# rakhimovv/lvt

Hardware: AMD Instinct MI355X
Metric: video-clips/sec/node (VQVAE+DSFVT train step, BAIR 64x64x16) (higher is better)
Workload: dtype f32

## Files before the change

lvt_amd/csrc/epilogue_fast.h:

```cpp
#pragma once
#include "lvt_common.h"

typedef float lvt_f32x16 __attribute__((ext_vector_type(16)));

template <int TM, int TN>
__device__ __forceinline__ void lvt_f16x2_finish(lvt_f32x16 (&acc)[TM][TN], lvt_f32x16 (&acx)[TM][TN], int unscale) {
    if (unscale >= -100 && unscale <= 120) {
        const float s = __uint_as_float((unsigned)(unscale + 127) << 23), sx = __uint_as_float((unsigned)(unscale + 116) << 23);
#pragma unroll
        for (int i = 0; i < TM; ++i)
#pragma unroll
            for (int j = 0; j < TN; ++j) acc[i][j] = acx[i][j] * sx + acc[i][j] * s;
    } else {
#pragma unroll
        for (int i = 0; i < TM; ++i)
#pragma unroll
            for (int j = 0; j < TN; ++j)
#pragma unroll
                for (int r = 0; r < 16; ++r) acc[i][j][r] = ldexpf(fmaf(acx[i][j][r], 1.f / 2048.f, acc[i][j][r]), unscale);
    }
}

struct LvtEpi {
    int M, N;
    float *C; long long ldc;
    long long coff;
    float alpha; int flags;
    const float *bias; const float *res; long long ldr; const float *mask; long long ldm;
};

struct LvtRowIdentity {
    static constexpr int LANE_STEP = 1;
    __device__ __forceinline__ long long operator()(int row) const { return row; }
};

template <int F, int TM, int TN, class RM = LvtRowIdentity>
__device__ __forceinline__ float lvt_epi_fast_wave(const LvtEpi &e, lvt_f32x16 (&acc)[TM][TN], float *wave_tile, int m_w, int n_w,
                                                   int lane, const RM rm = RM()) {
#pragma clang fp contract(off)
    static_assert(TM == 2 && TN == 2, "64 x 64 sub-tiles");
    constexpr int SW = TN * 32;
    const int flags = F >= 0 ? F : e.flags;
    const bool f_bias = flags & LVT_EPI_BIAS, f_res = flags & LVT_EPI_RESIDUAL, f_relu = flags & LVT_EPI_RELU, f_mask = flags & LVT_EPI_MASK;
    const bool f_leaky = flags & LVT_EPI_LEAKY, f_lkm = flags & LVT_EPI_LEAKY_MASK;
    const int l31 = lane & 31, half = lane >> 5;
    const int c4 = lane & 15, r0 = lane >> 4;
    const int col = n_w + 4 * c4;
    const bool colok = col < e.N;
    float4 bias4 = make_float4(0.f, 0.f, 0.f, 0.f);
    if (f_bias && colok) bias4 = *reinterpret_cast<const float4 *>(e.bias + col);
    float am = 0.f;
    long long orow_all[TM][8];
    float4 rv_all[TM][8], mv_all[TM][8];
#pragma unroll
    for (int i = 0; i < TM; ++i) {
        const int row0 = m_w + i * 32 + r0;
#pragma unroll
        for (int u = 0; u < 8; ++u) orow_all[i][u] = rm(row0 + 4 * u);
    }
    auto request = [&](int i) {
        const int row0 = m_w + i * 32 + r0;
        if (f_res) {
            const float *rp = e.res + e.coff + col;
#pragma unroll
            for (int u = 0; u < 8; ++u)
                rv_all[i][u] = (colok && row0 + 4 * u < e.M) ? *reinterpret_cast<const float4 *>(rp + orow_all[i][u] * e.ldr) : make_float4(0.f, 0.f, 0.f, 0.f);
        }
        if (f_mask) {
            const float *mp = e.mask + e.coff + col;
#pragma unroll
            for (int u = 0; u < 8; ++u)
                mv_all[i][u] = (colok && row0 + 4 * u < e.M) ? *reinterpret_cast<const float4 *>(mp + orow_all[i][u] * e.ldm) : make_float4(0.f, 0.f, 0.f, 0.f);
        }
    };
#pragma unroll
    for (int i = 0; i < TM; ++i) request(i);
#pragma unroll
    for (int i = 0; i < TM; ++i) {
#pragma unroll
        for (int j = 0; j < TN; ++j)
#pragma unroll
            for (int r = 0; r < 16; ++r) wave_tile[((r & 3) + 8 * (r >> 2) + 4 * half) * SW + 32 * j + l31] = acc[i][j][r];
        const int row0 = m_w + i * 32 + r0;
        const long long (&orow)[8] = orow_all[i];
        const float4 (&rv)[8] = rv_all[i];
        const float4 (&mv)[8] = mv_all[i];
        float *cp = e.C + e.coff + col;
#pragma unroll
        for (int u = 0; u < 8; ++u) {
            float4 v = *reinterpret_cast<const float4 *>(&wave_tile[(r0 + 4 * u) * SW + 4 * c4]);
            v.x *= e.alpha; v.y *= e.alpha; v.z *= e.alpha; v.w *= e.alpha;
            if (f_bias) { v.x += bias4.x; v.y += bias4.y; v.z += bias4.z; v.w += bias4.w; }
            if (f_res) { v.x += rv[u].x; v.y += rv[u].y; v.z += rv[u].z; v.w += rv[u].w; }
            if (f_relu) { v.x = fmaxf(v.x, 0.f); v.y = fmaxf(v.y, 0.f); v.z = fmaxf(v.z, 0.f); v.w = fmaxf(v.w, 0.f); }
            if (f_leaky) { v.x = lvt_leakyf(v.x); v.y = lvt_leakyf(v.y); v.z = lvt_leakyf(v.z); v.w = lvt_leakyf(v.w); }
            if (f_mask) { v.x = lvt_maskf(v.x, mv[u].x, f_lkm); v.y = lvt_maskf(v.y, mv[u].y, f_lkm); v.z = lvt_maskf(v.z, mv[u].z, f_lkm); v.w = lvt_maskf(v.w, mv[u].w, f_lkm); }
            if (colok && row0 + 4 * u < e.M) {
                am = fmaxf(am, fmaxf(fmaxf(lvt_absf(v.x), lvt_absf(v.y)), fmaxf(lvt_absf(v.z), lvt_absf(v.w))));
                *reinterpret_cast<float4 *>(cp + orow[u] * e.ldc) = v;
            }
        }
    }
    return am;
}

typedef __attribute__((address_space(1))) char lvt_gchar;
typedef float lvt_f32x4 __attribute__((ext_vector_type(4)));
typedef __attribute__((address_space(1))) lvt_f32x4 lvt_gf32x4;
__device__ __forceinline__ lvt_gchar *lvt_sgpr_ptr(lvt_gchar *p) { asm("" : "+s"(p)); return p; }
template <int F, int TM, int TN, class RM>
__device__ __forceinline__ float lvt_epi_lean_wave(const LvtEpi &e, lvt_f32x16 (&acc)[TM][TN], float *wave_tile, int m_w, int n_w, int lane,
                                                   const RM rm) {
#pragma clang fp contract(off)
    static_assert(F >= 0 && TM == 2 && TN == 2, "compile-time flags, 64 x 64 sub-tiles");
    constexpr int SW = TN * 32;
    constexpr bool f_bias = F & LVT_EPI_BIAS, f_res = F & LVT_EPI_RESIDUAL, f_relu = F & LVT_EPI_RELU, f_mask = F & LVT_EPI_MASK;
    constexpr bool f_leaky = F & LVT_EPI_LEAKY, f_lkm = F & LVT_EPI_LEAKY_MASK;
    const int l31 = lane & 31, half = lane >> 5;
    const int c4 = lane & 15, r0 = lane >> 4;
    const unsigned loff = (unsigned)(RM::LANE_STEP * r0) * (unsigned)e.ldc * 4u + 16u * c4;
    const unsigned ld4 = (unsigned)e.ldc * 4u;
    const long long first = (e.coff + n_w + rm(m_w) * e.ldc) * 4;
    lvt_f32x4 bias4 = {0.f, 0.f, 0.f, 0.f};
    if (f_bias) bias4 = *(const lvt_gf32x4 *)((lvt_gchar *)(e.bias + n_w) + 16u * c4);
    unsigned rowb[TM][8];
#pragma unroll
    for (int i = 0; i < TM; ++i)
#pragma unroll
        for (int u = 0; u < 8; ++u) rowb[i][u] = (unsigned)(rm(m_w + 32 * i + 4 * u) - rm(m_w)) * ld4;
    lvt_gchar *Cb = (lvt_gchar *)e.C + first;
    lvt_gchar *Rb = f_res ? (lvt_gchar *)e.res + first : nullptr;
    lvt_gchar *Mb = f_mask ? (lvt_gchar *)e.mask + first : nullptr;
    lvt_f32x4 rv[TM][8], mv[TM][8];
#pragma unroll
    for (int i = 0; i < TM; ++i) {
        if (f_res) {
#pragma unroll
            for (int u = 0; u < 8; ++u) rv[i][u] = *(const lvt_gf32x4 *)(lvt_sgpr_ptr(Rb + rowb[i][u]) + loff);
        }
        if (f_mask) {
#pragma unroll
            for (int u = 0; u < 8; ++u) mv[i][u] = *(const lvt_gf32x4 *)(lvt_sgpr_ptr(Mb + rowb[i][u]) + loff);
        }
    }
    auto key = [](float x) { return (__float_as_uint(x) << 1) + (1u << 24); };
    unsigned am = 1u << 24;
#pragma unroll
    for (int i = 0; i < TM; ++i) {
#pragma unroll
        for (int j = 0; j < TN; ++j)
#pragma unroll
            for (int r = 0; r < 16; ++r) wave_tile[((r & 3) + 8 * (r >> 2) + 4 * half) * SW + 32 * j + l31] = acc[i][j][r];
#pragma unroll
        for (int u = 0; u < 8; ++u) {
            lvt_f32x4 v = *reinterpret_cast<const lvt_f32x4 *>(&wave_tile[(r0 + 4 * u) * SW + 4 * c4]);
            if (f_bias) v += bias4;
            if (f_res) v += rv[i][u];
            if (f_relu) { v.x = fmaxf(v.x, 0.f); v.y = fmaxf(v.y, 0.f); v.z = fmaxf(v.z, 0.f); v.w = fmaxf(v.w, 0.f); }
            if (f_leaky) { v.x = lvt_leakyf(v.x); v.y = lvt_leakyf(v.y); v.z = lvt_leakyf(v.z); v.w = lvt_leakyf(v.w); }
            if (f_mask) { v.x = lvt_maskf(v.x, mv[i][u].x, f_lkm); v.y = lvt_maskf(v.y, mv[i][u].y, f_lkm); v.z = lvt_maskf(v.z, mv[i][u].z, f_lkm); v.w = lvt_maskf(v.w, mv[i][u].w, f_lkm); }
            am = max(max(am, key(v.x)), key(v.y));
            am = max(max(am, key(v.z)), key(v.w));
            *(lvt_gf32x4 *)(lvt_sgpr_ptr(Cb + rowb[i][u]) + loff) = v;
        }
    }
    return __uint_as_float((am - (1u << 24)) >> 1);
}

__device__ __forceinline__ bool lvt_epi_lean_ok(const LvtEpi &e) {
    return e.alpha == 1.f && (unsigned long long)e.ldc < (1ull << 20) && (!(e.flags & LVT_EPI_RESIDUAL) || e.ldr == e.ldc) &&
           (!(e.flags & LVT_EPI_MASK) || e.ldm == e.ldc);
}
template <int F, int TM, int TN, class RM = LvtRowIdentity>
__device__ __forceinline__ float lvt_epi_fast_pick(const LvtEpi &e, lvt_f32x16 (&acc)[TM][TN], float *wave_tile, int m_w, int n_w, int lane,
                                                   const RM rm = RM()) {
    if constexpr (F >= 0) {
        const int m_u = __builtin_amdgcn_readfirstlane(m_w), n_u = __builtin_amdgcn_readfirstlane(n_w);
        if (lvt_epi_lean_ok(e) && m_u + TM * 32 <= e.M && n_u + TN * 32 <= e.N)
            return lvt_epi_lean_wave<F, TM, TN, RM>(e, acc, wave_tile, m_u, n_u, lane, rm);
    }
    return lvt_epi_fast_wave<F, TM, TN, RM>(e, acc, wave_tile, m_w, n_w, lane, rm);
}

template <int TM, int TN, class RM = LvtRowIdentity>
__device__ __forceinline__ float lvt_epi_fast_dispatch(const LvtEpi &e, lvt_f32x16 (&acc)[TM][TN], float *wave_tile, int m_w, int n_w, int lane,
                                                       const RM rm = RM()) {
#define LVT_EPI_CASE(F) case (F): return lvt_epi_fast_pick<(F), TM, TN, RM>(e, acc, wave_tile, m_w, n_w, lane, rm)
    switch (e.flags & (LVT_EPI_BIAS | LVT_EPI_RESIDUAL | LVT_EPI_RELU | LVT_EPI_MASK | LVT_EPI_LEAKY | LVT_EPI_LEAKY_MASK)) {
    LVT_EPI_CASE(0);
    LVT_EPI_CASE(LVT_EPI_BIAS);
    LVT_EPI_CASE(LVT_EPI_BIAS | LVT_EPI_RELU);
    LVT_EPI_CASE(LVT_EPI_BIAS | LVT_EPI_RESIDUAL);
    LVT_EPI_CASE(LVT_EPI_BIAS | LVT_EPI_RESIDUAL | LVT_EPI_RELU);
    LVT_EPI_CASE(LVT_EPI_RESIDUAL);
    LVT_EPI_CASE(LVT_EPI_MASK);
    LVT_EPI_CASE(LVT_EPI_RESIDUAL | LVT_EPI_MASK);
    LVT_EPI_CASE(LVT_EPI_BIAS | LVT_EPI_LEAKY);
    LVT_EPI_CASE(LVT_EPI_MASK | LVT_EPI_LEAKY_MASK);
    default: return lvt_epi_fast_wave<-1, TM, TN, RM>(e, acc, wave_tile, m_w, n_w, lane, rm);
    }
#undef LVT_EPI_CASE
}

__device__ __forceinline__ unsigned lvt_amax_peek(const float *dst) {
    return (dst && threadIdx.x == 0) ? __hip_atomic_load(reinterpret_cast<const unsigned *>(dst), __ATOMIC_RELAXED, __HIP_MEMORY_SCOPE_AGENT) : 0u;
}
__device__ __forceinline__ void lvt_block_amax_commit_seen(float m, float *dst, float *scratch, unsigned seen) {
#pragma unroll
    for (int d = 32; d > 0; d >>= 1) m = fmaxf(m, __shfl_xor(m, d, 64));
    const int nw = (blockDim.x + 63) >> 6;
    if ((threadIdx.x & 63) == 0) scratch[threadIdx.x >> 6] = m;
    __syncthreads();
    if (threadIdx.x == 0) {
        for (int w = 1; w < nw; ++w) m = fmaxf(m, scratch[w]);
        const unsigned bits = __float_as_uint(m);
        if (bits > seen) atomicMax(reinterpret_cast<unsigned *>(dst), bits);
    }
}
```

lvt_amd/csrc/gemm_engine.hip:

```cpp
#include "lvt_common.h"
#include "epilogue_fast.h"
#include <string.h>
#include <stdlib.h>
#include <stdint.h>
#include <type_traits>

typedef float f32x16 __attribute__((ext_vector_type(16)));

#define BK 32
#define NTHREADS 256

enum { A_KPLAIN = 0, A_MPLAIN = 1, A_CONV_K = 2, A_CONVT_K = 3, A_CONV_M = 4, A_ONEHOT_M = 5, A_PATCH = 6, A_PATCHT = 7 };
enum { B_KPLAIN = 0, B_NPLAIN = 1, B_CONVT_W = 2 };

struct KParams {
    int M, N, K;
    const float *A; long long lda; int a_kb; long long a_skb;
    const float *B; long long ldb; int b_kb; long long b_skb;
    float *C; long long ldc; long long c_plane;
    int batch_inner;
    long long sA_o, sA_i, sB_o, sB_i, sC_o, sC_i;
    float alpha; int flags;
    const float *bias; const float *res; long long ldr; const float *mask; long long ldm;
    int splits; int k_per_split; float *partial; long long partial_stride;
// ... 630 lines not shown
            long long orow = row;
            if (AMODE == A_PATCH) orow = patch_orow(row);
            if (AMODE == A_PATCHT) orow = patcht_orow(row, cls);
            if (AMODE == A_CONVT_K) {
                const lvt_conv_geom &g = p.g;
                int m = row;
                const int qw = m % p.Wq; m /= p.Wq;
                const int qh = m % p.Hq; m /= p.Hq;
                const int qt = m % p.Tq; const int n = m / p.Tq;
                orow = (((long long)n * g.Ti + (g.st * qt + rt)) * g.Hi + (g.sh * qh + rh)) * g.Wi +
                       (g.sw * qw + rw);
            }
#pragma unroll
            for (int j = 0; j < TN; ++j) {
                const int col = n0 + wn * (TN * 32) + j * 32 + l31;
                if (col >= p.N) continue;
                float v = acc[i][j][r];
                if (p.splits > 1) {
                    p.partial[split * p.partial_stride + (long long)z * p.M * p.N + orow * p.N + col] = v;
                    continue;
                }
                v *= p.alpha;
                if (flags & LVT_EPI_BIAS) v += p.bias[col];
                if (flags & LVT_EPI_RESIDUAL) v += p.res[coff + orow * p.ldr + col];
                if (flags & LVT_EPI_RELU) v = fmaxf(v, 0.f);
                if (flags & LVT_EPI_LEAKY) v = lvt_leakyf(v);
                if (flags & LVT_EPI_TANH) v = tanhf(v);
                if (flags & LVT_EPI_SIGMOID) v = lvt_sigmoid_col(v, col < p.N - LVT_EPI_PAD_OF(flags));
                if (flags & LVT_EPI_MASK) v = lvt_maskf(v, p.mask[coff + orow * p.ldm + col], flags & LVT_EPI_LEAKY_MASK);
                float *cp = p.C + coff + orow * p.ldc + col;
                if (flags & LVT_EPI_ACCUM) v += *cp;
                *cp = v;
                am = fmaxf(am, lvt_absf(v));
            }
        }
    }
    if (p.c_amax && p.splits <= 1) {
        __shared__ float amax_scratch[8];
        lvt_block_amax_commit(am, p.c_amax, amax_scratch);
    }
}

struct TileCtx { int m0, n0, z, split, cls, kbeg, kend; const float *A, *B; long long coff; };
template <int AMODE, int BM, int BN>
__device__ __forceinline__ TileCtx lvt_tile_ctx(const KParams &p) {
    TileCtx t;
    const int ntn = (p.N + BN - 1) / BN;
    int wg = blockIdx.x;
    t.split = blockIdx.z;
    t.z = blockIdx.y;
    if (p.splits > 1 && ((gridDim.y * gridDim.z) & 7) == 0) {
        const unsigned lin = blockIdx.x + gridDim.x * (blockIdx.y + gridDim.y * blockIdx.z);
        const unsigned xcd = lin & 7, slot = lin >> 3;
        const unsigned grp = xcd + 8 * (slot / gridDim.x);
        t.z = (int)(grp % gridDim.y);
        t.split = (int)(grp / gridDim.y);
        wg = (int)(slot % gridDim.x);
    } else {
        const int nwg = gridDim.x, q = nwg >> 3, r = nwg & 7;
        const int xcd = wg & 7, slot = wg >> 3;
        wg = (xcd < r ? xcd * (q + 1) : r * (q + 1) + (xcd - r) * q) + slot;
    }
    t.n0 = (wg % ntn) * BN; t.m0 = (wg / ntn) * BM;
    t.A = p.A; t.B = p.B; t.coff = 0; t.cls = 0;
    if (AMODE == A_CONVT_K) {
        t.cls = t.z;
    } else {
        const int zo = t.z / p.batch_inner, zi = t.z % p.batch_inner;
        t.A += zo * p.sA_o + zi * p.sA_i;
        t.B += zo * p.sB_o + zi * p.sB_i;
        t.coff = zo * p.sC_o + zi * p.sC_i;
    }
    t.kbeg = 0; t.kend = p.K;
    if (p.splits > 1) {
        t.kbeg = t.split * p.k_per_split;
        t.kend = min(p.K, t.kbeg + p.k_per_split);
    }
    if (p.flags & LVT_CAUSAL_KMAX) t.kend = min(t.kend, t.m0 + BM);
    if (p.flags & LVT_CAUSAL_KMIN) t.kbeg = max(t.kbeg, (t.m0 / BK) * BK);
    if ((p.flags & LVT_CAUSAL_TILE) && t.n0 > t.m0 + BM - 1) t.kend = t.kbeg;
    return t;
}

template <int AMODE, int BM, int BN, int WM, int WN>
__device__ __forceinline__ void lvt_epilogue_vec(const KParams &p, f32x16 (&acc)[BM / WM / 32][BN / WN / 32], float *lds,
                                                 int m0, int n0, int wm, int wn, int lane, int cls, long long coff, int z,
                                                 int split) {
#pragma clang fp contract(off)
    constexpr int TM = BM / WM / 32, TN = BN / WN / 32;
    constexpr int SW = TN * 32;
    constexpr int C4 = SW / 4;
    const int l31 = lane & 31, half = lane >> 5;
    float *tile = lds + (wm * WN + wn) * (32 * SW);
    int rt = 0, rh = 0, rw = 0;
    if (AMODE == A_CONVT_K) {
        const lvt_conv_geom &g = p.g;
        const int fw = cls % g.sw, fh = (cls / g.sw) % g.sh, ft = cls / (g.sw * g.sh);
        rt = ((ft - g.pt) % g.st + g.st) % g.st;
        rh = ((fh - g.ph) % g.sh + g.sh) % g.sh;
        rw = ((fw - g.pw) % g.sw + g.sw) % g.sw;
    }
    const int flags = p.flags;
    const bool lkm = flags & LVT_EPI_LEAKY_MASK;
    float am = 0.f;
#pragma unroll
    for (int i = 0; i < TM; ++i) {
#pragma unroll
        for (int j = 0; j < TN; ++j)
#pragma unroll
            for (int r = 0; r < 16; ++r) tile[((r & 3) + 8 * (r >> 2) + 4 * half) * SW + 32 * j + l31] = acc[i][j][r];
        __syncthreads();
        if (AMODE != A_KPLAIN && AMODE != A_MPLAIN && p.splits <= 1 && (flags & LVT_EPI_MASK) &&
            !(flags & (LVT_EPI_PLANES | LVT_EPI_ACCUM | LVT_EPI_LEAKY | LVT_EPI_LEAKY_MASK))) {
            constexpr int NU = 32 * C4 / 64;
            long long oaddr[NU];
            int ocol[NU];
#pragma unroll
            for (int u = 0; u < NU; ++u) {
                const int idx = lane + 64 * u;
                const int rowl = idx / C4, c4 = idx % C4;
                const int row = m0 + wm * (TM * 32) + i * 32 + rowl;
                const int col = n0 + wn * SW + 4 * c4;
                ocol[u] = col;
                long long orow = -1;
                if (row < p.M && col < p.N) {
                    orow = row;
                    if (AMODE == A_PATCH) orow = patch_orow(row);
                    if (AMODE == A_PATCHT) orow = patcht_orow(row, cls);
                    if (AMODE == A_CONVT_K) {
                        const lvt_conv_geom &g = p.g;
                        int m = row;
                        const int qw = m % p.Wq; m /= p.Wq;
                        const int qh = m % p.Hq; m /= p.Hq;
                        const int qt = m % p.Tq; const int n = m / p.Tq;
                        orow = (((long long)n * g.Ti + (g.st * qt + rt)) * g.Hi + (g.sh * qh + rh)) * g.Wi + (g.sw * qw + rw);
                    }
                }
                oaddr[u] = orow;
            }
            float4 rv[NU], mv[NU];
            if (flags & LVT_EPI_RESIDUAL) {
#pragma unroll
                for (int u = 0; u < NU; ++u) rv[u] = oaddr[u] >= 0 ? ldg4(p.res + coff + oaddr[u] * p.ldr + ocol[u]) : zero4();
            } else {
#pragma unroll
                for (int u = 0; u < NU; ++u) rv[u] = zero4();
            }
#pragma unroll
            for (int u = 0; u < NU; ++u) mv[u] = oaddr[u] >= 0 ? ldg4(p.mask + coff + oaddr[u] * p.ldm + ocol[u]) : zero4();
#pragma unroll
            for (int u = 0; u < NU; ++u) {
                const int idx = lane + 64 * u;
                const int rowl = idx / C4, c4 = idx % C4;
                const int col = ocol[u];
                const long long orow = oaddr[u];
                if (orow >= 0) {
                    float4 v = *reinterpret_cast<const float4 *>(&tile[rowl * SW + 4 * c4]);
                    v.x *= p.alpha; v.y *= p.alpha; v.z *= p.alpha; v.w *= p.alpha;
                    if (flags & LVT_EPI_BIAS) { const float4 b = ldg4(p.bias + col); v.x += b.x; v.y += b.y; v.z += b.z; v.w += b.w; }
                    v.x += rv[u].x; v.y += rv[u].y; v.z += rv[u].z; v.w += rv[u].w;
                    if (flags & LVT_EPI_RELU) { v.x = fmaxf(v.x, 0.f); v.y = fmaxf(v.y, 0.f); v.z = fmaxf(v.z, 0.f); v.w = fmaxf(v.w, 0.f); }
                    if (flags & LVT_EPI_TANH) { v.x = tanhf(v.x); v.y = tanhf(v.y); v.z = tanhf(v.z); v.w = tanhf(v.w); }
                    if (flags & LVT_EPI_SIGMOID) {
                        const int nr = p.N - LVT_EPI_PAD_OF(flags) - col;
                        v.x = lvt_sigmoid_col(v.x, nr > 0); v.y = lvt_sigmoid_col(v.y, nr > 1); v.z = lvt_sigmoid_col(v.z, nr > 2); v.w = lvt_sigmoid_col(v.w, nr > 3);
                    }
                    v.x = mv[u].x > 0.f ? v.x : 0.f; v.y = mv[u].y > 0.f ? v.y : 0.f; v.z = mv[u].z > 0.f ? v.z : 0.f; v.w = mv[u].w > 0.f ? v.w : 0.f;
                    am = fmaxf(am, fmaxf(fmaxf(lvt_absf(v.x), lvt_absf(v.y)), fmaxf(lvt_absf(v.z), lvt_absf(v.w))));
                    *reinterpret_cast<float4 *>(p.C + coff + orow * p.ldc + col) = v;
                }
            }
        } else {
#pragma unroll
            for (int u = 0; u < 32 * C4 / 64; ++u) {
                const int idx = lane + 64 * u;
                const int rowl = idx / C4, c4 = idx % C4;
                const int row = m0 + wm * (TM * 32) + i * 32 + rowl;
                const int col = n0 + wn * SW + 4 * c4;
                if (row < p.M && col < p.N) {
                    float4 v = *reinterpret_cast<const float4 *>(&tile[rowl * SW + 4 * c4]);
                    long long orow = row;
                    if (AMODE == A_PATCH) orow = patch_orow(row);
                    if (AMODE == A_PATCHT) orow = patcht_orow(row, cls);
                    if (AMODE == A_CONVT_K) {
                        const lvt_conv_geom &g = p.g;
                        int m = row;
                        const int qw = m % p.Wq; m /= p.Wq;
                        const int qh = m % p.Hq; m /= p.Hq;
                        const int qt = m % p.Tq; const int n = m / p.Tq;
                        orow = (((long long)n * g.Ti + (g.st * qt + rt)) * g.Hi + (g.sh * qh + rh)) * g.Wi + (g.sw * qw + rw);
                    }
                    if (p.splits > 1) {
                        *reinterpret_cast<float4 *>(p.partial + split * p.partial_stride + (long long)z * p.M * p.N + orow * p.N + col) = v;
// ... 159 lines not shown
                        acx[i][j] = __builtin_amdgcn_mfma_f32_32x32x16_f16(a[1][i], b[0][j], acx[i][j], 0, 0, 0);
            }
        } else {
            const unsigned short *Arh[TM], *Brh[TN];
#pragma unroll
            for (int i = 0; i < TM; ++i) Arh[i] = Ah + hrow<BM>(wm * (TM * 32) + i * 32 + l31) + 8 * half;
#pragma unroll
            for (int j = 0; j < TN; ++j) Brh[j] = Bh + hrow<BN>(wn * (TN * 32) + j * 32 + l31) + 8 * half;
#pragma unroll
            for (int ks = 0; ks < BK; ks += 16) {
                bf16x8 a[3][TM], b[3][TN];
#pragma unroll
                for (int q = 0; q < 3; ++q) {
#pragma unroll
                    for (int i = 0; i < TM; ++i)
                        a[q][i] = *reinterpret_cast<const bf16x8 *>(Arh[i] + q * PSA + ks);
#pragma unroll
                    for (int j = 0; j < TN; ++j)
                        b[q][j] = *reinterpret_cast<const bf16x8 *>(Brh[j] + q * PSB + ks);
                }
                constexpr int TA[6] = {1, 0, 2, 0, 1, 0}, TB[6] = {1, 2, 0, 1, 0, 0};
#pragma unroll
                for (int t = 0; t < 6; ++t)
#pragma unroll
                    for (int i = 0; i < TM; ++i)
#pragma unroll
                        for (int j = 0; j < TN; ++j)
                            acc[i][j] = __builtin_amdgcn_mfma_f32_32x32x16_bf16(a[TA[t]][i], b[TB[t]][j], acc[i][j], 0, 0, 0);
            }
        }
        __syncthreads();
        if (has_next) {
            if (MATH == 0) { al.store(As); bl.store(Bs); }
            else if (MATH == 1) { al.store_split(Ah); bl.store_split(Bh); }
            else { al.store_split2(Ah, sa); bl.store_split2(Bh, sb); }
        }
        __syncthreads();
    }
    if constexpr (MATH == 2) lvt_f16x2_finish<TM, TN>(acc, acx, unscale);

    if constexpr (COLSUM) {
        if (bl.sum_on) bl.write_colsum(lds, p.colsum_partial + (long long)split * p.N, n0, p.N, tid);
    }
    if constexpr (COLSUM_A) {
        if (al.sum_on) al.write_colsum(lds, p.colsum_partial + ((long long)split * gridDim.y + z) * p.M, m0, p.M, tid);
    }
    if constexpr (AMODE != A_CONVT_K && TM == 2 && TN == 2 && LDS_FLOATS >= TURN_FLOATS + 16) {
        if (p.vec_epi && !(p.flags & (LVT_EPI_PLANES | LVT_EPI_ACCUM | LVT_EPI_TANH | LVT_EPI_SIGMOID))) {
            LvtEpi e;
            e.M = p.M; e.N = p.N;
            float *wave_tile = lds + wave * (32 * TN * 32);
            if (COLSUM || COLSUM_A) __syncthreads();
            if (p.splits > 1) {
                e.C = p.partial; e.ldc = p.N; e.coff = split * p.partial_stride + (long long)z * p.M * p.N; e.alpha = 1.f; e.flags = 0;
                e.bias = nullptr; e.res = nullptr; e.ldr = 0; e.mask = nullptr; e.ldm = 0;
                (void)lvt_epi_fast_pick<0, TM, TN>(e, acc, wave_tile, m0 + wm * (TM * 32), n0 + wn * (TN * 32), lane);
                return;
            }
            const unsigned seen = lvt_amax_peek(p.c_amax);
            e.C = p.C; e.ldc = p.ldc; e.coff = coff; e.alpha = p.alpha; e.flags = p.flags;
            e.bias = p.bias; e.res = p.res; e.ldr = p.ldr; e.mask = p.mask; e.ldm = p.ldm;
            const float am_w = lvt_epi_fast_dispatch<TM, TN>(e, acc, wave_tile, m0 + wm * (TM * 32), n0 + wn * (TN * 32), lane);
            if (p.c_amax) lvt_block_amax_commit_seen(am_w, p.c_amax, lds + TURN_FLOATS, seen);
            return;
        }
    }
    if (p.vec_epi) lvt_epilogue_vec<AMODE, BM, BN, WM, WN>(p, acc, lds, m0, n0, wm, wn, lane, cls, coff, z, split);
    else lvt_epilogue<AMODE, BM, BN, WM, WN>(p, acc, m0, n0, wm, wn, l31, half, cls, coff, z, split);
}

#define PT_PW 18
#define PT_PIX (PT_PW * PT_PW)
#define PT_PLANE (PT_PIX * HLD)
#define PT_THREADS 512
typedef __attribute__((address_space(3))) void pt_lds_void;
typedef __attribute__((address_space(1))) const void pt_gl_void;
#define PT_BIMG_BYTES (2 * HPlane<128>::SIZE * 2)
template <int MODE, int MATH, int BIMG = 0>
__global__ __launch_bounds__(PT_THREADS) void lvt_conv_patch_kernel(const KParams p) {
    static_assert(!BIMG || MATH == 2, "weight images are f16x2 planes");
    constexpr int BM = 256, BN = 128, WM = 4, WN = 2, TM = 2, TN = 2;
    constexpr int NTAPS = MODE == 0 ? 9 : 4;
    constexpr int NP = MATH == 2 ? 2 : 3;
    constexpr int PSB = HPlane<BN>::SIZE;
    constexpr bool DBLA = MATH == 2;
    constexpr int A_IMG = NP * PT_PLANE;
    constexpr int A_BYTES = A_IMG * 2 * (DBLA ? 2 : 1), B_BYTES = NP * PSB * 2;
    constexpr int STAGE_FLOATS = (A_BYTES + 2 * B_BYTES) / 4 + 8;
    constexpr int TURN_FLOATS = WM * WN * 32 * (TN * 32);
    constexpr int LDS_FLOATS = STAGE_FLOATS > TURN_FLOATS ? STAGE_FLOATS : TURN_FLOATS;
    __shared__ __attribute__((aligned(16))) float lds[LDS_FLOATS];
    unsigned short *Ah = reinterpret_cast<unsigned short *>(lds);
    unsigned short *Bh0 = Ah + A_IMG * (DBLA ? 2 : 1);
    int unscale = 0;
    float sa = 1.f, sb = 1.f;
    if (MATH == 2) { sa = lvt_f16_scale(p.a_amax, unscale); sb = lvt_f16_scale(p.b_amax, unscale); }

    const int tid = threadIdx.x, lane = tid & 63, wave = tid >> 6;
    const int wm = wave / WN, wn = wave % WN;
    const int l31 = lane & 31, half = lane >> 5;
    const int Ci = p.g.Ci;
    const int ntn = p.N / BN;
    int wg = blockIdx.x;
    {
        const int nwg = gridDim.x, q = nwg >> 3, r = nwg & 7;
        const int xcd = wg & 7, slot = wg >> 3;
        wg = (xcd < r ? xcd * (q + 1) : r * (q + 1) + (xcd - r) * q) + slot;
    }
    const int n0 = (wg % ntn) * BN;
    const int frame = MODE == 1 ? (wg / ntn) >> 2 : wg / ntn, phase = MODE == 1 ? (wg / ntn) & 3 : 0, m0 = frame * BM;
    const float *xf = p.A + (long long)frame * (MODE == 2 ? 1024 : 256) * Ci;

    constexpr int PWALK = MODE == 2 ? 17 : PT_PW;
    constexpr int PUNITS = PWALK * PWALK * 8, PPASS = (PUNITS + PT_THREADS - 1) / PT_THREADS;
    float4 pv[PPASS];
    auto patch_fetch = [&](int chunk) {
#pragma unroll
        for (int j = 0; j < PPASS; ++j) {
            const int u = tid + PT_THREADS * j;
            const int pp = u >> 3, q = u & 7;
            const int py = pp / PWALK, px = pp - py * PWALK;
            if (MODE == 2) {
                const int iy = 2 * py + ((chunk >> 1) & 1) - 1, ix = 2 * px + (chunk & 1) - 1;
                const bool ok = u < PUNITS && (unsigned)iy < 32u && (unsigned)ix < 32u;
                pv[j] = ok ? ldg4(xf + (iy * 32 + ix) * Ci + (chunk >> 2) * 32 + q * 4) : zero4();
            } else {
                const bool ok = u < PUNITS && (unsigned)(py - 1) < 16u && (unsigned)(px - 1) < 16u;
                const float *src = xf + ((py - 1) * 16 + (px - 1)) * Ci + chunk * 32 + q * 4;
                pv[j] = ok ? ldg4(src) : zero4();
            }
        }
    };
    auto patch_store = [&](unsigned short *img) {
#pragma unroll
        for (int j = 0; j < PPASS; ++j) {
            const int u = tid + PT_THREADS * j;
            if (u < PUNITS) {
                const int pp = u >> 3;
                unsigned short *d = img + (MODE == 2 ? pp + pp / PWALK : pp) * HLD + (u & 7) * 4;
                if (MATH == 2) {
                    uint2 ph, pl;
                    split2(pv[j], sa, ph, pl);
                    *reinterpret_cast<uint2 *>(d) = ph;
                    *reinterpret_cast<uint2 *>(d + PT_PLANE) = pl;
                } else {
                    uint2 p1, p2, p3;
                    split3(pv[j], p1, p2, p3);
                    *reinterpret_cast<uint2 *>(d) = p1;
                    *reinterpret_cast<uint2 *>(d + PT_PLANE) = p2;
                    *reinterpret_cast<uint2 *>(d + 2 * PT_PLANE) = p3;
                }
            }
        }
    };
    const bool bact = tid < 256;
    const int bkk0 = (tid >> 5) & 7, bnq = tid & 31;
    const float *bcol = p.B + n0 + bnq * 4;
    float4 bv[4];
    auto b_fetch = [&](int step) {
        const int cc = step / NTAPS, tap = step - cc * NTAPS;
        const int wrow = MODE == 2 ? ((cc & 3) * NTAPS + tap) * Ci + (cc >> 2) * 32 : (phase * NTAPS + tap) * Ci + cc * 32;
        const float *src = bcol + (long long)(wrow + bkk0 * 4) * p.ldb;
#pragma unroll
        for (int i = 0; i < 4; ++i) bv[i] = ldg4(src + (long long)i * p.ldb);
    };

    f32x16 acc[TM][TN];
    f32x16 acx[MATH == 2 ? TM : 1][MATH == 2 ? TN : 1];
#pragma unroll
    for (int i = 0; i < TM; ++i)
#pragma unroll
        for (int j = 0; j < TN; ++j)
#pragma unroll
            for (int r = 0; r < 16; ++r) {
                acc[i][j][r] = 0.f;
                if (MATH == 2) acx[i][j][r] = 0.f;
            }
    auto b_store = [&](unsigned short *dst) {
        if (MATH == 2) store_split2_block<BN>(dst, bnq * 4, bkk0 * 4, bv, sb);
        else store_split_block<BN>(dst, bnq * 4, bkk0 * 4, bv);
    };
    const int wave_s = __builtin_amdgcn_readfirstlane(wave);
    constexpr int B_UNITS = PT_BIMG_BYTES / 16;
    static_assert(PT_BIMG_BYTES == NP * PSB * 2 || !BIMG, "image = the LDS buffer");
    const char *bimg0 = BIMG ? p.b_img + (long long)(n0 / BN) * PT_BIMG_BYTES + tid * 16 : nullptr;
    auto b_dma = [&](int step, unsigned short *dst) {
        const int cc = step / NTAPS, tap = step - cc * NTAPS;
        const int wrow = MODE == 2 ? ((cc & 3) * NTAPS + tap) * Ci + (cc >> 2) * 32 : (phase * NTAPS + tap) * Ci + cc * 32;
        const char *src = bimg0 + (long long)(wrow >> 5) * ntn * PT_BIMG_BYTES;
        char *d = reinterpret_cast<char *>(dst) + wave_s * 1024;
        __builtin_amdgcn_global_load_lds((pt_gl_void *)src, (pt_lds_void *)d, 16, 0, 0);
        __builtin_amdgcn_global_load_lds((pt_gl_void *)(src + 8192), (pt_lds_void *)(d + 8192), 16, 0, 0);
        if (tid + 1024 < B_UNITS) __builtin_amdgcn_global_load_lds((pt_gl_void *)(src + 16384), (pt_lds_void *)(d + 16384), 16, 0, 0);
    };
    const int b_nprobe = wave_s * 64 + 1024 < B_UNITS ? 3 : 2;
    const unsigned b_probe = (unsigned)((lane % b_nprobe) * 8192 + wave_s * 1024 + (lane & 31) * 16);
    auto b_landed = [&](const unsigned short *dst) {
        asm volatile("s_waitcnt vmcnt(0)" ::: "memory");
        const int v = *reinterpret_cast<const volatile int *>(reinterpret_cast<const char *>(dst) + b_probe);
        (void)v;
        asm volatile("s_waitcnt lgkmcnt(0)" ::: "memory");
    };

    int arow[TM];
    {
        const int q = l31 >> 2, e = l31 & 3;
        const int yy = __popc(q) & 1, x = 4 * (q >> 1) + e;
#pragma unroll
        for (int i = 0; i < TM; ++i) arow[i] = ((2 * (2 * wm + i) + yy) * PT_PW + x) * HLD + 8 * half;
    }
    int brow[TN];
#pragma unroll
    for (int j = 0; j < TN; ++j) brow[j] = hrow<BN>(wn * (TN * 32) + j * 32 + l31) + 8 * half;

    const int nchunks = (Ci / 32) * (MODE == 2 ? 4 : 1), nsteps = nchunks * NTAPS;
    patch_fetch(0);
    if (BIMG) b_dma(0, Bh0);
    else if (bact) b_fetch(0);
    patch_store(Ah);
    if (BIMG) b_landed(Bh0);
    else if (bact) b_store(Bh0);
    __syncthreads();

    for (int step = 0; step < nsteps; ++step) {
        const int cc = step / NTAPS, tap = step - cc * NTAPS;
        const bool has_next = step + 1 < nsteps;
        const bool new_chunk = has_next && tap == NTAPS - 1;
        if (BIMG) { if (has_next) b_dma(step + 1, Bh0 + ((step + 1) & 1) * (NP * PSB)); }
        else if (has_next && bact) b_fetch(step + 1);
        if (DBLA ? (cc + 1 < nchunks && tap == NTAPS - 2) : new_chunk) patch_fetch(cc + 1);
        const unsigned short *Bh = Bh0 + (step & 1) * (NP * PSB);
        const unsigned short *Acur = Ah + (DBLA ? (cc & 1) * A_IMG : 0);
        const unsigned short *Ap = MODE == 0 ? Acur + ((tap / 3) * PT_PW + (tap % 3)) * HLD
                                             : Acur + (((phase >> 1) + (tap >> 1)) * PT_PW + (phase & 1) + (tap & 1)) * HLD;
        if constexpr (MATH == 2) {
#pragma unroll
            for (int ks = 0; ks < BK; ks += 16) {
                f16x8 a[2][TM], b[2][TN];
#pragma unroll
                for (int q = 0; q < 2; ++q) {
#pragma unroll
                    for (int i = 0; i < TM; ++i) a[q][i] = *reinterpret_cast<const f16x8 *>(Ap + arow[i] + q * PT_PLANE + ks);
#pragma unroll
                    for (int j = 0; j < TN; ++j) b[q][j] = *reinterpret_cast<const f16x8 *>(Bh + brow[j] + q * PSB + ks);
                }
#pragma unroll
                for (int i = 0; i < TM; ++i)
#pragma unroll
                    for (int j = 0; j < TN; ++j)
                        acx[i][j] = __builtin_amdgcn_mfma_f32_32x32x16_f16(a[0][i], b[1][j], acx[i][j], 0, 0, 0);
#pragma unroll
                for (int i = 0; i < TM; ++i)
#pragma unroll
                    for (int j = 0; j < TN; ++j)
                        acc[i][j] = __builtin_amdgcn_mfma_f32_32x32x16_f16(a[0][i], b[0][j], acc[i][j], 0, 0, 0);
#pragma unroll
                for (int i = 0; i < TM; ++i)
#pragma unroll
                    for (int j = 0; j < TN; ++j)
                        acx[i][j] = __builtin_amdgcn_mfma_f32_32x32x16_f16(a[1][i], b[0][j], acx[i][j], 0, 0, 0);
            }
            if (DBLA && new_chunk) patch_store(Ah + ((cc + 1) & 1) * A_IMG);
        } else {
#pragma unroll
            for (int ks = 0; ks < BK; ks += 16) {
                bf16x8 a[3][TM], b[3][TN];
#pragma unroll
                for (int q = 0; q < 3; ++q) {
#pragma unroll
                    for (int i = 0; i < TM; ++i) a[q][i] = *reinterpret_cast<const bf16x8 *>(Ap + arow[i] + q * PT_PLANE + ks);
#pragma unroll
                    for (int j = 0; j < TN; ++j) b[q][j] = *reinterpret_cast<const bf16x8 *>(Bh + brow[j] + q * PSB + ks);
                }
                constexpr int TA[6] = {1, 0, 2, 0, 1, 0}, TB[6] = {1, 2, 0, 1, 0, 0};
#pragma unroll
                for (int t = 0; t < 6; ++t)
#pragma unroll
                    for (int i = 0; i < TM; ++i)
#pragma unroll
                        for (int j = 0; j < TN; ++j)
                            acc[i][j] = __builtin_amdgcn_mfma_f32_32x32x16_bf16(a[TA[t]][i], b[TB[t]][j], acc[i][j], 0, 0, 0);
            }
        }
        if (!BIMG && has_next && bact) b_store(Bh0 + ((step + 1) & 1) * (NP * PSB));
        if (!DBLA && new_chunk) {
            __syncthreads();
            patch_store(Ah);
        }
        if (BIMG && has_next) b_landed(Bh0 + ((step + 1) & 1) * (NP * PSB));
        __syncthreads();
    }
    if constexpr (MATH == 2) lvt_f16x2_finish<TM, TN>(acc, acx, unscale);
    if (p.vec_epi && p.splits <= 1 && !(p.flags & (LVT_EPI_PLANES | LVT_EPI_ACCUM | LVT_EPI_TANH | LVT_EPI_SIGMOID))) {
        const unsigned seen = lvt_amax_peek(p.c_amax);
        LvtEpi e;
        e.M = p.M; e.N = p.N; e.C = p.C; e.ldc = p.ldc; e.coff = 0; e.alpha = p.alpha; e.flags = p.flags;
        e.bias = p.bias; e.res = p.res; e.ldr = p.ldr; e.mask = p.mask; e.ldm = p.ldm;
        float *wave_tile = lds + wave * (32 * TN * 32);
        float am_w;
        if (MODE != 1) am_w = lvt_epi_fast_dispatch<TM, TN, PatchRows>(e, acc, wave_tile, m0 + wm * (TM * 32), n0 + wn * (TN * 32), lane, PatchRows());
        else am_w = lvt_epi_fast_dispatch<TM, TN, PatchTRows>(e, acc, wave_tile, m0 + wm * (TM * 32), n0 + wn * (TN * 32), lane, PatchTRows{phase});
        if (p.c_amax) lvt_block_amax_commit_seen(am_w, p.c_amax, lds + TURN_FLOATS, seen);
        return;
    }
    if (MODE != 1) lvt_epilogue_vec<A_PATCH, BM, BN, WM, WN>(p, acc, lds, m0, n0, wm, wn, lane, 0, 0, 0, 0);
    else lvt_epilogue_vec<A_PATCHT, BM, BN, WM, WN>(p, acc, lds, m0, n0, wm, wn, lane, phase, 0, 0, 0);
}

#define WIDE_THREADS 512
#define WT_PA (256 + 32)
#define WT_PB (128 + 32)
typedef short s16x4 __attribute__((ext_vector_type(4)));
__device__ __forceinline__ f16x8 wide_tr_frag(const unsigned short *p, int pitch4) {
    typedef __attribute__((address_space(3))) s16x4 lds_v4;
    const s16x4 lo = __builtin_amdgcn_ds_read_tr16_b64_v4i16((lds_v4 *)(p));
    const s16x4 hi = __builtin_amdgcn_ds_read_tr16_b64_v4i16((lds_v4 *)(p + pitch4));
    union { struct { s16x4 a, b; } s; f16x8 v; } u;
    u.s.a = lo; u.s.b = hi;
    return u.v;
}
template <int TA, int TB>
__global__ __launch_bounds__(WIDE_THREADS, 2) void lvt_gemm_wide_kernel(const KParams p) {
    constexpr int BM = 256, BN = 128, WM = 4, WN = 2, TM = 2, TN = 2;
    constexpr int AMODE = TA ? A_MPLAIN : A_KPLAIN;
    constexpr int PA = WT_PA, PB = WT_PB;
    constexpr int PSA = TA ? BK * PA : HPlane<BM>::SIZE, PSB = TB ? BK * PB : HPlane<BN>::SIZE;
    constexpr int STAGE = 2 * (PSA + PSB);
    static_assert(PA % 4 == 0 && PB % 4 == 0 && PSA % 8 == 0 && PSB % 8 == 0, "transposing reads need 8-byte aligned addresses");
    static_assert(BK * PA <= HPlane<BM>::SIZE && BK * PB <= HPlane<BN>::SIZE, "the memory-order images are the smaller ones");
    constexpr int STAGE_FLOATS = (2 * STAGE) / 2 + 8;
    constexpr int TURN_FLOATS = WM * WN * 32 * (TN * 32);
    constexpr int LDS_FLOATS = STAGE_FLOATS > TURN_FLOATS ? STAGE_FLOATS : TURN_FLOATS;
    __shared__ __attribute__((aligned(16))) float lds[LDS_FLOATS];
    unsigned short *S0 = reinterpret_cast<unsigned short *>(lds);

    const int tid = threadIdx.x, lane = tid & 63, wave = tid >> 6;
    const int wm = wave / WN, wn = wave % WN;
    const int l31 = lane & 31, half = lane >> 5;
    const TileCtx tc = lvt_tile_ctx<AMODE, BM, BN>(p);
    const int m0 = tc.m0, n0 = tc.n0, kbeg = tc.kbeg, kend = tc.kend;

    int unscale = 0;
    const float sa = lvt_f16_scale(p.a_amax, unscale, p.a_amax2), sb = lvt_f16_scale(p.b_amax, unscale, p.b_amax2);

    float4 av[4], bv[2];
    const int r0 = tid >> 3, kq = tid & 7;
    const int kk0 = TA ? tid >> 6 : 0, mq = tid & 63;
    const int bkk0 = tid >> 5, bnq = tid & 31;
    const char *Ak = reinterpret_cast<const char *>(tc.A), *Bk = reinterpret_cast<const char *>(tc.B);
    unsigned aoff[4], boff_g[2];
    int a_kin = 0, b_kin = 0;
    if (!TA) {
#pragma unroll
        for (int i = 0; i < 4; ++i) aoff[i] = (unsigned)(((long long)min(m0 + r0 + 64 * i, p.M - 1) * p.lda + kq * 4) * 4);
        const int blk = kbeg / p.a_kb;
        a_kin = kbeg - blk * p.a_kb;
        Ak += ((long long)blk * p.a_skb + a_kin) * 4;
    } else {
        const int m = m0 + mq * 4;
#pragma unroll
        for (int i = 0; i < 4; ++i) aoff[i] = (unsigned)(((long long)(kk0 * 4 + i) * p.lda + (m < p.M ? m : 0)) * 4);
        Ak += (long long)kbeg * p.lda * 4;
    }
    if (!TB) {
#pragma unroll
        for (int i = 0; i < 2; ++i) boff_g[i] = (unsigned)(((long long)min(n0 + r0 + 64 * i, p.N - 1) * p.ldb + kq * 4) * 4);
        const int blk = kbeg / p.b_kb;
        b_kin = kbeg - blk * p.b_kb;
        Bk += ((long long)blk * p.b_skb + b_kin) * 4;
    } else {
        const int n = n0 + bnq * 4;
#pragma unroll
        for (int i = 0; i < 2; ++i) boff_g[i] = (unsigned)(((long long)(bkk0 * 2 + i) * p.ldb + (n < p.N ? n : 0)) * 4);
        Bk += (long long)kbeg * p.ldb * 4;
    }
    const bool sum_on = TA && p.colsum_partial != nullptr && n0 == 0;
    float4 colacc = zero4();
    auto fetch = [&]() {
#pragma unroll
        for (int i = 0; i < 4; ++i) av[i] = *reinterpret_cast<const float4 *>(Ak + aoff[i]);
        if (!TA) {
            a_kin += BK;
            const bool wrap = a_kin >= p.a_kb;
            Ak += wrap ? ((long long)p.a_skb - p.a_kb + BK) * 4 : (long long)BK * 4;
            a_kin = wrap ? 0 : a_kin;
        } else {
            Ak += (long long)BK * p.lda * 4;
            if (sum_on) {
#pragma unroll
// ... 1032 lines not shown
```

Baseline: 1399.

## Use 16x16x32 MFMA blocks in f16x2 patch conv GEMM with matching epilogue layout

In the MATH==2 (split-f16) path of the patch convolution kernel, each 32x32x16 MFMA k-step pair is replaced by 16x16x32 MFMAs over four sub-blocks per 32x32 accumulator, with new per-lane A/B row offsets. The epilogue LDS transpose gains a SHAPE template parameter so the 16x16 accumulator register layout is scattered correctly before the vectorized store. The aim is to use the shorter-latency or denser 16x16x32 instruction with a single k-tile load per step. The cost is more instructions, accumulator element shuffling around each MFMA, and a risk of extra register moves.

```diff
diff --git a/lvt_amd/csrc/epilogue_fast.h b/lvt_amd/csrc/epilogue_fast.h
--- a/lvt_amd/csrc/epilogue_fast.h
+++ b/lvt_amd/csrc/epilogue_fast.h
@@ -34,7 +34,35 @@
     __device__ __forceinline__ long long operator()(int row) const { return row; }
 };
 
-template <int F, int TM, int TN, class RM = LvtRowIdentity>
+template <int SHAPE, int TN>
+__device__ __forceinline__ void lvt_turn_store(float *wave_tile, const lvt_f32x16 (&acc_i)[TN], int lane) {
+    constexpr int SW = TN * 32;
+    if constexpr (SHAPE == 32) {
+        const int l31 = lane & 31, half = lane >> 5;
+#pragma unroll
+        for (int j = 0; j < TN; ++j)
+#pragma unroll
+            for (int r = 0; r < 16; ++r) wave_tile[((r & 3) + 8 * (r >> 2) + 4 * half) * SW + 32 * j + l31] = acc_i[j][r];
+    } else {
+        static_assert(SHAPE == 16, "MFMA block shape");
+        const int g = lane >> 4, c = lane & 15;
+        const int po = g >> 1, odd = (g ^ po) & 1;
+        const int colp = c < 8 ? c : c < 12 ? c + 4 : c - 4;
+#pragma unroll
+        for (int h = 0; h < 2; ++h)
+#pragma unroll
+            for (int r = 0; r < 4; ++r) {
+                const int q = 2 * (r >> 1) + 4 * po + (((r >> 1) ^ po ^ h) & 1);
+                float *d = wave_tile + (4 * q + 2 * (r & 1) + odd) * SW + colp;
+#pragma unroll
+                for (int j = 0; j < TN; ++j)
+#pragma unroll
+                    for (int jj = 0; jj < 2; ++jj) d[32 * j + 16 * jj] = acc_i[j][4 * (2 * h + jj) + r];
+            }
+    }
+}
+
+template <int F, int TM, int TN, class RM = LvtRowIdentity, int SHAPE = 32>
 __device__ __forceinline__ float lvt_epi_fast_wave(const LvtEpi &e, lvt_f32x16 (&acc)[TM][TN], float *wave_tile, int m_w, int n_w,
                                                    int lane, const RM rm = RM()) {
 #pragma clang fp contract(off)
@@ -43,7 +71,6 @@
     const int flags = F >= 0 ? F : e.flags;
     const bool f_bias = flags & LVT_EPI_BIAS, f_res = flags & LVT_EPI_RESIDUAL, f_relu = flags & LVT_EPI_RELU, f_mask = flags & LVT_EPI_MASK;
     const bool f_leaky = flags & LVT_EPI_LEAKY, f_lkm = flags & LVT_EPI_LEAKY_MASK;
-    const int l31 = lane & 31, half = lane >> 5;
     const int c4 = lane & 15, r0 = lane >> 4;
     const int col = n_w + 4 * c4;
     const bool colok = col < e.N;
@@ -77,10 +104,7 @@
     for (int i = 0; i < TM; ++i) request(i);
 #pragma unroll
     for (int i = 0; i < TM; ++i) {
-#pragma unroll
-        for (int j = 0; j < TN; ++j)
-#pragma unroll
-            for (int r = 0; r < 16; ++r) wave_tile[((r & 3) + 8 * (r >> 2) + 4 * half) * SW + 32 * j + l31] = acc[i][j][r];
+        lvt_turn_store<SHAPE, TN>(wave_tile, acc[i], lane);
         const int row0 = m_w + i * 32 + r0;
         const long long (&orow)[8] = orow_all[i];
         const float4 (&rv)[8] = rv_all[i];
@@ -108,7 +132,7 @@
 typedef float lvt_f32x4 __attribute__((ext_vector_type(4)));
 typedef __attribute__((address_space(1))) lvt_f32x4 lvt_gf32x4;
 __device__ __forceinline__ lvt_gchar *lvt_sgpr_ptr(lvt_gchar *p) { asm("" : "+s"(p)); return p; }
-template <int F, int TM, int TN, class RM>
+template <int F, int TM, int TN, class RM, int SHAPE = 32>
 __device__ __forceinline__ float lvt_epi_lean_wave(const LvtEpi &e, lvt_f32x16 (&acc)[TM][TN], float *wave_tile, int m_w, int n_w, int lane,
                                                    const RM rm) {
 #pragma clang fp contract(off)
@@ -116,7 +140,6 @@
     constexpr int SW = TN * 32;
     constexpr bool f_bias = F & LVT_EPI_BIAS, f_res = F & LVT_EPI_RESIDUAL, f_relu = F & LVT_EPI_RELU, f_mask = F & LVT_EPI_MASK;
     constexpr bool f_leaky = F & LVT_EPI_LEAKY, f_lkm = F & LVT_EPI_LEAKY_MASK;
-    const int l31 = lane & 31, half = lane >> 5;
     const int c4 = lane & 15, r0 = lane >> 4;
     const unsigned loff = (unsigned)(RM::LANE_STEP * r0) * (unsigned)e.ldc * 4u + 16u * c4;
     const unsigned ld4 = (unsigned)e.ldc * 4u;
@@ -147,10 +170,7 @@
     unsigned am = 1u << 24;
 #pragma unroll
     for (int i = 0; i < TM; ++i) {
-#pragma unroll
-        for (int j = 0; j < TN; ++j)
-#pragma unroll
-            for (int r = 0; r < 16; ++r) wave_tile[((r & 3) + 8 * (r >> 2) + 4 * half) * SW + 32 * j + l31] = acc[i][j][r];
+        lvt_turn_store<SHAPE, TN>(wave_tile, acc[i], lane);
 #pragma unroll
         for (int u = 0; u < 8; ++u) {
             lvt_f32x4 v = *reinterpret_cast<const lvt_f32x4 *>(&wave_tile[(r0 + 4 * u) * SW + 4 * c4]);
@@ -171,21 +191,21 @@
     return e.alpha == 1.f && (unsigned long long)e.ldc < (1ull << 20) && (!(e.flags & LVT_EPI_RESIDUAL) || e.ldr == e.ldc) &&
            (!(e.flags & LVT_EPI_MASK) || e.ldm == e.ldc);
 }
-template <int F, int TM, int TN, class RM = LvtRowIdentity>
+template <int F, int TM, int TN, class RM = LvtRowIdentity, int SHAPE = 32>
 __device__ __forceinline__ float lvt_epi_fast_pick(const LvtEpi &e, lvt_f32x16 (&acc)[TM][TN], float *wave_tile, int m_w, int n_w, int lane,
                                                    const RM rm = RM()) {
     if constexpr (F >= 0) {
         const int m_u = __builtin_amdgcn_readfirstlane(m_w), n_u = __builtin_amdgcn_readfirstlane(n_w);
         if (lvt_epi_lean_ok(e) && m_u + TM * 32 <= e.M && n_u + TN * 32 <= e.N)
-            return lvt_epi_lean_wave<F, TM, TN, RM>(e, acc, wave_tile, m_u, n_u, lane, rm);
-    }
-    return lvt_epi_fast_wave<F, TM, TN, RM>(e, acc, wave_tile, m_w, n_w, lane, rm);
-}
-
-template <int TM, int TN, class RM = LvtRowIdentity>
+            return lvt_epi_lean_wave<F, TM, TN, RM, SHAPE>(e, acc, wave_tile, m_u, n_u, lane, rm);
+    }
+    return lvt_epi_fast_wave<F, TM, TN, RM, SHAPE>(e, acc, wave_tile, m_w, n_w, lane, rm);
+}
+
+template <int TM, int TN, class RM = LvtRowIdentity, int SHAPE = 32>
 __device__ __forceinline__ float lvt_epi_fast_dispatch(const LvtEpi &e, lvt_f32x16 (&acc)[TM][TN], float *wave_tile, int m_w, int n_w, int lane,
                                                        const RM rm = RM()) {
-#define LVT_EPI_CASE(F) case (F): return lvt_epi_fast_pick<(F), TM, TN, RM>(e, acc, wave_tile, m_w, n_w, lane, rm)
+#define LVT_EPI_CASE(F) case (F): return lvt_epi_fast_pick<(F), TM, TN, RM, SHAPE>(e, acc, wave_tile, m_w, n_w, lane, rm)
     switch (e.flags & (LVT_EPI_BIAS | LVT_EPI_RESIDUAL | LVT_EPI_RELU | LVT_EPI_MASK | LVT_EPI_LEAKY | LVT_EPI_LEAKY_MASK)) {
     LVT_EPI_CASE(0);
     LVT_EPI_CASE(LVT_EPI_BIAS);
@@ -197,7 +217,7 @@
     LVT_EPI_CASE(LVT_EPI_RESIDUAL | LVT_EPI_MASK);
     LVT_EPI_CASE(LVT_EPI_BIAS | LVT_EPI_LEAKY);
     LVT_EPI_CASE(LVT_EPI_MASK | LVT_EPI_LEAKY_MASK);
-    default: return lvt_epi_fast_wave<-1, TM, TN, RM>(e, acc, wave_tile, m_w, n_w, lane, rm);
+    default: return lvt_epi_fast_wave<-1, TM, TN, RM, SHAPE>(e, acc, wave_tile, m_w, n_w, lane, rm);
     }
 #undef LVT_EPI_CASE
 }
diff --git a/lvt_amd/csrc/gemm_engine.hip b/lvt_amd/csrc/gemm_engine.hip
--- a/lvt_amd/csrc/gemm_engine.hip
+++ b/lvt_amd/csrc/gemm_engine.hip
@@ -736,7 +736,7 @@
     return t;
 }
 
-template <int AMODE, int BM, int BN, int WM, int WN>
+template <int AMODE, int BM, int BN, int WM, int WN, int SHAPE = 32>
 __device__ __forceinline__ void lvt_epilogue_vec(const KParams &p, f32x16 (&acc)[BM / WM / 32][BN / WN / 32], float *lds,
                                                  int m0, int n0, int wm, int wn, int lane, int cls, long long coff, int z,
                                                  int split) {
@@ -744,7 +744,6 @@
     constexpr int TM = BM / WM / 32, TN = BN / WN / 32;
     constexpr int SW = TN * 32;
     constexpr int C4 = SW / 4;
-    const int l31 = lane & 31, half = lane >> 5;
     float *tile = lds + (wm * WN + wn) * (32 * SW);
     int rt = 0, rh = 0, rw = 0;
     if (AMODE == A_CONVT_K) {
@@ -759,10 +758,7 @@
     float am = 0.f;
 #pragma unroll
     for (int i = 0; i < TM; ++i) {
-#pragma unroll
-        for (int j = 0; j < TN; ++j)
-#pragma unroll
-            for (int r = 0; r < 16; ++r) tile[((r & 3) + 8 * (r >> 2) + 4 * half) * SW + 32 * j + l31] = acc[i][j][r];
+        lvt_turn_store<SHAPE, TN>(tile, acc[i], lane);
         __syncthreads();
         if (AMODE != A_KPLAIN && AMODE != A_MPLAIN && p.splits <= 1 && (flags & LVT_EPI_MASK) &&
             !(flags & (LVT_EPI_PLANES | LVT_EPI_ACCUM | LVT_EPI_LEAKY | LVT_EPI_LEAKY_MASK))) {
@@ -1088,6 +1084,7 @@
     constexpr int BM = 256, BN = 128, WM = 4, WN = 2, TM = 2, TN = 2;
     constexpr int NTAPS = MODE == 0 ? 9 : 4;
     constexpr int NP = MATH == 2 ? 2 : 3;
+    constexpr int SHAPE = MATH == 2 ? 16 : 32;
     constexpr int PSB = HPlane<BN>::SIZE;
     constexpr bool DBLA = MATH == 2;
     constexpr int A_IMG = NP * PT_PLANE;
@@ -1218,6 +1215,16 @@
     int brow[TN];
 #pragma unroll
     for (int j = 0; j < TN; ++j) brow[j] = hrow<BN>(wn * (TN * 32) + j * 32 + l31) + 8 * half;
+    int arow16[2 * TM], brow16[2 * TN];
+    {
+        const int a = lane & 15, g = a >> 2, koct = ((lane >> 4) & 1) * 2 + (lane >> 5);
+        const int x = 2 * (a & 3) + (g == 0 ? 0 : g == 1 ? 1 : g == 2 ? 9 : 8);
+        const int n = a < 8 ? a : a < 12 ? a + 4 : a - 4;
+#pragma unroll
+        for (int ib = 0; ib < 2 * TM; ++ib) arow16[ib] = ((2 * TM * wm + ib) * PT_PW + x) * HLD + 8 * koct;
+#pragma unroll
+        for (int jb = 0; jb < 2 * TN; ++jb) brow16[jb] = hrow<BN>(wn * (TN * 32) + jb * 16 + n) + 8 * koct;
+    }
 
     const int nchunks = (Ci / 32) * (MODE == 2 ? 4 : 1), nsteps = nchunks * NTAPS;
     patch_fetch(0);
@@ -1240,32 +1247,32 @@
         const unsigned short *Ap = MODE == 0 ? Acur + ((tap / 3) * PT_PW + (tap % 3)) * HLD
                                              : Acur + (((phase >> 1) + (tap >> 1)) * PT_PW + (phase & 1) + (tap & 1)) * HLD;
         if constexpr (MATH == 2) {
-#pragma unroll
-            for (int ks = 0; ks < BK; ks += 16) {
-                f16x8 a[2][TM], b[2][TN];
-#pragma unroll
-                for (int q = 0; q < 2; ++q) {
-#pragma unroll
-                    for (int i = 0; i < TM; ++i) a[q][i] = *reinterpret_cast<const f16x8 *>(Ap + arow[i] + q * PT_PLANE + ks);
-#pragma unroll
-                    for (int j = 0; j < TN; ++j) b[q][j] = *reinterpret_cast<const f16x8 *>(Bh + brow[j] + q * PSB + ks);
-                }
-#pragma unroll
-                for (int i = 0; i < TM; ++i)
-#pragma unroll
-                    for (int j = 0; j < TN; ++j)
-                        acx[i][j] = __builtin_amdgcn_mfma_f32_32x32x16_f16(a[0][i], b[1][j], acx[i][j], 0, 0, 0);
-#pragma unroll
-                for (int i = 0; i < TM; ++i)
-#pragma unroll
-                    for (int j = 0; j < TN; ++j)
-                        acc[i][j] = __builtin_amdgcn_mfma_f32_32x32x16_f16(a[0][i], b[0][j], acc[i][j], 0, 0, 0);
-#pragma unroll
-                for (int i = 0; i < TM; ++i)
-#pragma unroll
-                    for (int j = 0; j < TN; ++j)
-                        acx[i][j] = __builtin_amdgcn_mfma_f32_32x32x16_f16(a[1][i], b[0][j], acx[i][j], 0, 0, 0);
-            }
+            static_assert(BK == 32, "one 16x16x32 MFMA per block and k-tile");
+            f16x8 a[2][2 * TM], b[2][2 * TN];
+#pragma unroll
+            for (int q = 0; q < 2; ++q) {
+#pragma unroll
+                for (int ib = 0; ib < 2 * TM; ++ib) a[q][ib] = *reinterpret_cast<const f16x8 *>(Ap + arow16[ib] + q * PT_PLANE);
+#pragma unroll
+                for (int jb = 0; jb < 2 * TN; ++jb) b[q][jb] = *reinterpret_cast<const f16x8 *>(Bh + brow16[jb] + q * PSB);
+            }
+            auto mfma16 = [](const f16x8 av, const f16x8 bv, f32x16 &t, const int s) {
+                lvt_f32x4 c = {t[s], t[s + 1], t[s + 2], t[s + 3]};
+                c = __builtin_amdgcn_mfma_f32_16x16x32_f16(av, bv, c, 0, 0, 0);
+                t[s] = c[0]; t[s + 1] = c[1]; t[s + 2] = c[2]; t[s + 3] = c[3];
+            };
+#pragma unroll
+            for (int ib = 0; ib < 2 * TM; ++ib)
+#pragma unroll
+                for (int jb = 0; jb < 2 * TN; ++jb) mfma16(a[0][ib], b[1][jb], acx[ib >> 1][jb >> 1], 4 * (2 * (ib & 1) + (jb & 1)));
+#pragma unroll
+            for (int ib = 0; ib < 2 * TM; ++ib)
+#pragma unroll
+                for (int jb = 0; jb < 2 * TN; ++jb) mfma16(a[0][ib], b[0][jb], acc[ib >> 1][jb >> 1], 4 * (2 * (ib & 1) + (jb & 1)));
+#pragma unroll
+            for (int ib = 0; ib < 2 * TM; ++ib)
+#pragma unroll
+                for (int jb = 0; jb < 2 * TN; ++jb) mfma16(a[1][ib], b[0][jb], acx[ib >> 1][jb >> 1], 4 * (2 * (ib & 1) + (jb & 1)));
             if (DBLA && new_chunk) patch_store(Ah + ((cc + 1) & 1) * A_IMG);
         } else {
 #pragma unroll
@@ -1304,13 +1311,13 @@
         e.bias = p.bias; e.res = p.res; e.ldr = p.ldr; e.mask = p.mask; e.ldm = p.ldm;
         float *wave_tile = lds + wave * (32 * TN * 32);
         float am_w;
-        if (MODE != 1) am_w = lvt_epi_fast_dispatch<TM, TN, PatchRows>(e, acc, wave_tile, m0 + wm * (TM * 32), n0 + wn * (TN * 32), lane, PatchRows());
-        else am_w = lvt_epi_fast_dispatch<TM, TN, PatchTRows>(e, acc, wave_tile, m0 + wm * (TM * 32), n0 + wn * (TN * 32), lane, PatchTRows{phase});
+        if (MODE != 1) am_w = lvt_epi_fast_dispatch<TM, TN, PatchRows, SHAPE>(e, acc, wave_tile, m0 + wm * (TM * 32), n0 + wn * (TN * 32), lane, PatchRows());
+        else am_w = lvt_epi_fast_dispatch<TM, TN, PatchTRows, SHAPE>(e, acc, wave_tile, m0 + wm * (TM * 32), n0 + wn * (TN * 32), lane, PatchTRows{phase});
         if (p.c_amax) lvt_block_amax_commit_seen(am_w, p.c_amax, lds + TURN_FLOATS, seen);
         return;
     }
-    if (MODE != 1) lvt_epilogue_vec<A_PATCH, BM, BN, WM, WN>(p, acc, lds, m0, n0, wm, wn, lane, 0, 0, 0, 0);
-    else lvt_epilogue_vec<A_PATCHT, BM, BN, WM, WN>(p, acc, lds, m0, n0, wm, wn, lane, phase, 0, 0, 0);
+    if (MODE != 1) lvt_epilogue_vec<A_PATCH, BM, BN, WM, WN, SHAPE>(p, acc, lds, m0, n0, wm, wn, lane, 0, 0, 0, 0);
+    else lvt_epilogue_vec<A_PATCHT, BM, BN, WM, WN, SHAPE>(p, acc, lds, m0, n0, wm, wn, lane, phase, 0, 0, 0);
 }
 
 #define WIDE_THREADS 512
```

After: 1409 (median of 6 runs). About the same (+0.7%).
